# OSU-Bee-Lab/buzzdetect

Measured on AMD Instinct MI355X. Metric: yamnet_windows_per_s, higher is better.
Workload: dtype f32 (split-f16x3 MFMA products, f32 accumulate)

## Files before the change

buzzdetect_amd/csrc/sepchip.hip:

```cpp
#include "bd_device.h"

namespace bd {

namespace {

constexpr int kChipHalfBytes = 97 * 64;
constexpr int kChipSlotBytes = 2 * kChipHalfBytes;

constexpr int kChipMaxLayers = 5;
struct ChipChain {
    const float* dw_w[kChipMaxLayers];
    const float* dw_b[kChipMaxLayers];
    const _Float16* whi[kChipMaxLayers];
    const _Float16* wlo[kChipMaxLayers];
    const float* pw_u[kChipMaxLayers];
    const float* pw_b[kChipMaxLayers];
    const float* ndw_w;
    const _Float16 *w7hi, *w7lo;
    const float *u7, *b7;
};
template <typename T>
__device__ __forceinline__ const T* chain_ptr(int field, int li) {
    typedef const __attribute__((address_space(4))) unsigned long long* kptr;
    const kptr ka = (kptr)__builtin_amdgcn_kernarg_segment_ptr();
    return reinterpret_cast<const T*>(ka[field * kChipMaxLayers + li]);
}
static_assert(sizeof(ChipChain) == (6 * kChipMaxLayers + 5) * 8, "six tables of five pointers + five");

template <bool PLAIN, int NSLOT, bool TRACE = false, bool NDW = false, bool PLANES = false, bool PW7 = false>
__global__ __launch_bounds__(512, 2) void sep_chip_kernel(const ChipChain ch, const float* X, float* Y, int nl,
                                                           long long M, unsigned* __restrict__ range_flag,
                                                           unsigned long long* __restrict__ dbg = nullptr, int tune = 0) {
    static_assert(NSLOT >= 9 && NSLOT <= 16, "ring size");
    constexpr int K = 512, KQ = K / 16;
    constexpr int NPEND = 16 - NSLOT;
    extern __shared__ __attribute__((aligned(16))) char sm[];
    const int tid = threadIdx.x;
    const int lane = tid & 63;
    const int wc = __builtin_amdgcn_readfirstlane(tid >> 6);
    const int frow = lane & 31, fh = lane >> 5;
    const long long m0 = (long long)blockIdx.x * 96;
    float rmax = 0.0f;
    int tsn = 0;
#define CHIP_TS()                                                                                         \
    if constexpr (TRACE) {                                                                                \
        if (blockIdx.x == 0 && lane == 0 && (wc == 0 || wc == 5) && tsn < 64)                             \
            dbg[(wc == 5 ? 64 : 0) + tsn] = __builtin_amdgcn_s_memtime();                                 \
        ++tsn;                                                                                            \
    }
    CHIP_TS()

    const int wb0 = fh * (48 * 64 + 64) + ((frow >> 3) << 4) + 2 * (frow & 7);
    const int ra0 = frow * 64 + ((fh ^ ((frow >> 2) & 3)) << 4);
    const int ra1 = ra0 + 2048 + (frow >= 16 ? 64 : 0);
    const unsigned lane16 = lane * 16, c4 = frow * 4;

    f32x16 acc[3][2];
    unsigned pend[48], out0[48];

#define CHIP_DW(J, ST, TAPS)                                                                              \
    {                                                                                                     \
        float wt[9];                                                                                      \
        _Pragma("unroll") for (int t = 0; t < 9; ++t)                                                     \
            wt[t] = __builtin_bit_cast(float, __builtin_amdgcn_raw_buffer_load_b32(TAPS, c4, (t * K + 32 * (ST)) * 4, 0)); \
        const float shift = __builtin_bit_cast(float, __builtin_amdgcn_raw_buffer_load_b32(TAPS, c4, (9 * K + 32 * (ST)) * 4, 0)); \
        _Pragma("unroll") for (int y = 0; y < 6; ++y)                                                     \
            _Pragma("unroll") for (int x = 0; x < 4; ++x) {                                               \
                v2f a = {shift, shift};                                                                   \
                _Pragma("unroll") for (int kh = 0; kh < 3; ++kh)                                          \
                    _Pragma("unroll") for (int kw = 0; kw < 3; ++kw) {                                    \
                        const int iy = y + kh - 1, ix = x + kw - 1;                                       \
                        if (iy < 0 || iy >= 6 || ix < 0 || ix >= 4) continue;                             \
                        a = __builtin_elementwise_fma(in2[iy][ix], v2f{wt[kh * 3 + kw], wt[kh * 3 + kw]}, a); \
                    }                                                                                     \
                _Pragma("unroll") for (int w = 0; w < 2; ++w) {                                           \
                    const float v = fmaxf(w ? a.y : a.x, 0.0f);                                           \
                    unsigned pk = (unsigned)__builtin_bit_cast(unsigned short, (_Float16)v);              \
                     \
                     \
                    asm volatile("v_fma_mixhi_f16 %0, %0, -1.0, %2 op_sel:[0,0,0] op_sel_hi:[1,0,0]\n\tv_max_f32 %1, %1, %2" \
                                 : "+v"(pk), "+v"(rmax) : "v"(v));                                        \
                    const int rl = 24 * w + 4 * y + x;                                \
                    if ((J) == 1) pend[rl] = pk;                                                          \
                    else out0[rl] = pk;                                                                   \
                }                                                                                         \
            }                                                                                             \
    }
#define CHIP_PUBLISH()                                                                                    \
    {                                                                                                     \
        int wbl = wb0;        \
        asm volatile("" : "+v"(wbl));                       \
        char* const slot0 = sm + wc * kChipSlotBytes;                                                     \
        _Pragma("unroll") for (int rl = 0; rl < 48; ++rl) CHIP_PUT(slot0, rl, out0[rl])                   \
        if (wc + 8 < NSLOT) {                                                \
            char* const slot1 = sm + (wc + 8) * kChipSlotBytes;                                           \
            _Pragma("unroll") for (int rl = 0; rl < 48; ++rl) CHIP_PUT(slot1, rl, pend[rl])               \
        }                                                                                                 \
    }
#define CHIP_PUT(SLOT, RL, PK)                                                                            \
    {                                                                                                     \
        char* const p_ = (SLOT) + (wbl ^ ((((RL) >> 2) & 3) << 4)) + (RL) * 64;                           \
        *reinterpret_cast<unsigned short*>(p_) = (unsigned short)(PK);                                    \
        *reinterpret_cast<unsigned short*>(p_ + kChipHalfBytes) = (unsigned short)((PK) >> 16);           \
    }
#define CHIP_TAPS_RSRC(DW_W) __builtin_amdgcn_make_buffer_rsrc(const_cast<float*>(DW_W), 0, 10 * K * 4, 0x00020000)

    auto k_loop = [&](auto kq_c, const _Float16* const Wfhi, const _Float16* const Wflo) __attribute__((always_inline)) {
        constexpr int KQL = decltype(kq_c)::value;
        constexpr int NS = KQL / 2;
        constexpr int NP = NS > NSLOT ? NS - NSLOT : 0;
        static_assert(NP == 0 || NP == NPEND, "a layer of K = 512 or one that fits the ring");
        const __amdgpu_buffer_rsrc_t bhr = __builtin_amdgcn_make_buffer_rsrc(const_cast<_Float16*>(Wfhi), 0, 16 * KQL * K * 2, 0x00020000);
        const __amdgpu_buffer_rsrc_t blr = __builtin_amdgcn_make_buffer_rsrc(const_cast<_Float16*>(Wflo), 0, 16 * KQL * K * 2, 0x00020000);
        const int btile = wc * (KQL * 1024);
        constexpr int jstep = 8 * KQL * 1024;
        f16x8 bh0[2], bl0[2], bh1[2], bl1[2];
#define CHIP_LB(R, B, Q, J) B[J] = __builtin_bit_cast(f16x8, __builtin_amdgcn_raw_buffer_load_b128(R, lane16, btile + (J) * jstep + (Q) * 1024, 0));
#define CHIP_BLOAD(BH, BL, Q) { CHIP_LB(bhr, BH, Q, 0) CHIP_LB(blr, BL, Q, 0) CHIP_LB(bhr, BH, Q, 1) CHIP_LB(blr, BL, Q, 1) }
        CHIP_BLOAD(bh0, bl0, 0)
        __syncthreads();
        CHIP_TS()

        float zero;
        asm volatile("v_mov_b32 %0, 0" : "=v"(zero));
#pragma unroll
        for (int i = 0; i < 3; ++i)
#pragma unroll
            for (int j = 0; j < 2; ++j)
#pragma unroll
                for (int r = 0; r < 16; ++r) acc[i][j][r] = zero;
#define CHIP_LAH(A, S, I) A = *reinterpret_cast<const f16x8*>(abase + (((I) == 1 ? ra1 : ra0) ^ ((S) << 5)) + ((I) == 2 ? 4096 + 64 : 0));
#define CHIP_LAL(A, S, I) A = *reinterpret_cast<const f16x8*>(abase + (((I) == 1 ? ra1 : ra0) ^ ((S) << 5)) + ((I) == 2 ? 4096 + 64 : 0) + kChipHalfBytes);
#define CHIP_MF(I, J, A, B) acc[I][J] = __builtin_amdgcn_mfma_f32_32x32x16_f16(A, B, acc[I][J], 0, 0, 0);
#define CHIP_SB __builtin_amdgcn_sched_barrier(0);
#define CHIP_NOP
#define CHIP_STEP(I, AH, AL, BH, BL, M1, M2, M3, M4, M5, M6)                                              \
    if constexpr (!PLAIN) {                                                                               \
        CHIP_MF(I, 0, AL, BH[0]) M1 CHIP_SB                                                               \
        CHIP_MF(I, 0, AH, BL[0]) M2 CHIP_SB                                                               \
    } else {                                                                                              \
        M1 M2                                                                                             \
    }                                                                                                     \
    CHIP_MF(I, 0, AH, BH[0]) M3 CHIP_SB                                                                   \
    if constexpr (!PLAIN) {                                                                               \
        CHIP_MF(I, 1, AL, BH[1]) M4 CHIP_SB                                                               \
        CHIP_MF(I, 1, AH, BL[1]) M5 CHIP_SB                                                               \
    } else {                                                                                              \
        M4 M5                                                                                             \
    }                                                                                                     \
    CHIP_MF(I, 1, AH, BH[1]) M6 CHIP_SB
#define CHIP_STAGES(FROM, TO)                                                                             \
    if ((FROM) < (TO)) {                                                                                  \
        f16x8 ah0, al0, ah1, al1, ah2, al2;                                                               \
        const char* abase = sm + ((FROM) < NSLOT ? (FROM) : (FROM) - NSLOT) * kChipSlotBytes;             \
        CHIP_LAH(ah0, 0, 0) CHIP_LAL(al0, 0, 0) CHIP_LAH(ah1, 0, 1) CHIP_LAL(al1, 0, 1)                   \
        _Pragma("nounroll") for (int kk = (FROM); kk < (TO); ++kk) {                                      \
            const int q1 = 2 * kk + 1, q2 = 2 * kk + 2 < KQL ? 2 * kk + 2 : 0;     \
            const char* const anext = sm + (kk + 1 < (TO) ? (kk + 1 < NSLOT ? kk + 1 : kk + 1 - NSLOT) : (kk < NSLOT ? kk : kk - NSLOT)) * kChipSlotBytes; \
            CHIP_STEP(0, ah0, al0, bh0, bl0, CHIP_LB(bhr, bh1, q1, 0), CHIP_LB(blr, bl1, q1, 0), CHIP_LB(bhr, bh1, q1, 1),  \
                      CHIP_LB(blr, bl1, q1, 1), CHIP_LAH(ah2, 0, 2), CHIP_LAL(al2, 0, 2))                 \
            CHIP_STEP(1, ah1, al1, bh0, bl0, CHIP_LAH(ah0, 1, 0), CHIP_LAL(al0, 1, 0), CHIP_NOP, CHIP_NOP, CHIP_NOP, CHIP_NOP) \
            CHIP_STEP(2, ah2, al2, bh0, bl0, CHIP_LAH(ah1, 1, 1), CHIP_LAL(al1, 1, 1), CHIP_LB(blr, bl0, q2, 0),            \
                      CHIP_LB(bhr, bh0, q2, 0), CHIP_NOP, CHIP_LB(blr, bl0, q2, 1))                       \
            CHIP_STEP(0, ah0, al0, bh1, bl1, CHIP_LB(bhr, bh0, q2, 1), CHIP_LAH(ah2, 1, 2), CHIP_LAL(al2, 1, 2), CHIP_NOP, CHIP_NOP, CHIP_NOP) \
            abase = anext;          \
            CHIP_STEP(1, ah1, al1, bh1, bl1, CHIP_LAH(ah0, 0, 0), CHIP_LAL(al0, 0, 0), CHIP_NOP, CHIP_NOP, CHIP_NOP, CHIP_NOP) \
            CHIP_STEP(2, ah2, al2, bh1, bl1, CHIP_LAH(ah1, 0, 1), CHIP_LAL(al1, 0, 1), CHIP_NOP, CHIP_NOP, CHIP_NOP, CHIP_NOP) \
        }                                                                                                 \
    }
        CHIP_STAGES(0, NP)
        CHIP_TS()
        if constexpr (NP > 0) {
            __syncthreads();
            CHIP_TS()
            if (wc >= 8 - NPEND) {
                char* const slot = sm + (wc + 8 - NSLOT) * kChipSlotBytes;
                int wbl = wb0;
                asm volatile("" : "+v"(wbl));
#pragma unroll
                for (int rl = 0; rl < 48; ++rl) CHIP_PUT(slot, rl, pend[rl])
            }
        }
        CHIP_TS()
        if constexpr (NP > 0) __syncthreads();
        CHIP_TS()
        CHIP_STAGES(NP, NS)
        CHIP_TS()
#undef CHIP_STAGES
#undef CHIP_STEP
#undef CHIP_BLOAD
#undef CHIP_LB
#undef CHIP_LAH
#undef CHIP_LAL
#undef CHIP_MF
#undef CHIP_SB
#undef CHIP_NOP
    };

    auto next_layer = [&](const float* const taps_w, const float* const pu, const float* const pb) __attribute__((always_inline)) {
        const __amdgpu_buffer_rsrc_t taps = CHIP_TAPS_RSRC(taps_w);
        const __amdgpu_buffer_rsrc_t pur = __builtin_amdgcn_make_buffer_rsrc(const_cast<float*>(pu), 0, K * 4, 0x00020000);
        const __amdgpu_buffer_rsrc_t pbr = __builtin_amdgcn_make_buffer_rsrc(const_cast<float*>(pb), 0, K * 4, 0x00020000);
#pragma unroll
        for (int j = 0; j < 2; ++j) {
            const int st = j ? wc + 8 : wc;
            const float u = __builtin_bit_cast(float, __builtin_amdgcn_raw_buffer_load_b32(pur, c4, 128 * st, 0));
            const float b = __builtin_bit_cast(float, __builtin_amdgcn_raw_buffer_load_b32(pbr, c4, 128 * st, 0));
            float ev[12][4];
#pragma unroll
            for (int q = 0; q < 6; ++q)
#pragma unroll
                for (int x = 0; x < 4; ++x) {
                    const float a01 = fmaxf(fmaf(acc[q >> 2][j][4 * (q & 3) + x], u, b), 0.0f);
                    const float a23 = fmaxf(fmaf(acc[(q + 6) >> 2][j][4 * ((q + 6) & 3) + x], u, b), 0.0f);
                    const auto r = __builtin_amdgcn_permlane32_swap(__builtin_bit_cast(unsigned, a01),
                                                                    __builtin_bit_cast(unsigned, a23), false, false);
                    ev[2 * q][x] = __builtin_bit_cast(float, (unsigned)r[0]);
                    ev[2 * q + 1][x] = __builtin_bit_cast(float, (unsigned)r[1]);
                }
            v2f in2[6][4];
#pragma unroll
            for (int y = 0; y < 6; ++y)
#pragma unroll
                for (int x = 0; x < 4; ++x) in2[y][x] = v2f{ev[y][x], ev[6 + y][x]};
            if (j == 0) CHIP_DW(0, st, taps)
            else CHIP_DW(1, st, taps)
            CHIP_TS()
        }
        __syncthreads();
        CHIP_TS()
        CHIP_PUBLISH()
    };

    const long long rows_left = M - m0;
    const unsigned tile_bytes = (unsigned)(rows_left < 96 ? rows_left : 96) * (K * 4);
    if constexpr (PW7) {
        const long long w0 = m0 / 24, wleft = M / 24 - w0;
        const __amdgpu_buffer_rsrc_t pr = __builtin_amdgcn_make_buffer_rsrc(
            const_cast<char*>(reinterpret_cast<const char*>(X)) + (size_t)w0 * kDw7PlaneBytes, 0,
            (unsigned)(wleft < 4 ? wleft : 4) * kDw7PlaneBytes, 0x00020000);
        constexpr int kPieces = 8 * kChipSlotBytes / 1024;
        static_assert(kPieces * 1024 == 8 * kChipSlotBytes && 8 * kChipSlotBytes <= NSLOT * kChipSlotBytes, "whole pieces");
#pragma unroll
        for (int t = 0; t < (kPieces + 7) / 8; ++t) {
            const int n = 8 * t + wc;
            if (n >= kPieces) break;
            const int c = 64 * n + lane;
            const int s = c / (kChipSlotBytes / 16), cs = c - s * (kChipSlotBytes / 16);
            const int h = cs >= kChipHalfBytes / 16 ? 1 : 0;
            const int o = (cs - h * (kChipHalfBytes / 16)) * 16;
            const bool skew = o >= 48 * 64 && o < 49 * 64;
            const int rho = o < 48 * 64 ? o >> 6 : (o - 64) >> 6;
            const int p = (o >> 4) & 3, w = rho / 24;
            const unsigned src = (unsigned)(w * kDw7PlaneBytes + s * (kDw7PlaneBytes / 8) + h * (kDw7PlaneBytes / 16) +
                                            (rho - 24 * w) * 64 + ((p ^ ((rho >> 2) & 3)) << 4));
            const unsigned off = skew || (PLAIN && h) ? 0x7ffffff0u : src;
            __builtin_amdgcn_raw_ptr_buffer_load_lds(pr, (__attribute__((address_space(3))) void*)(sm + n * 1024), 16, off, 0, 0, 0);
        }
        asm volatile("s_waitcnt vmcnt(0)" ::: "memory");
        CHIP_TS()
        k_loop(std::integral_constant<int, 16>{}, ch.w7hi, ch.w7lo);
        next_layer(ch.dw_w[0], ch.u7, ch.b7);
    } else {
        const __amdgpu_buffer_rsrc_t xrs = __builtin_amdgcn_make_buffer_rsrc(const_cast<float*>(X) + (size_t)m0 * K, 0, tile_bytes, 0x00020000);
        const __amdgpu_buffer_rsrc_t taps0 = CHIP_TAPS_RSRC(ch.dw_w[0]);
        const unsigned xo = (48u * fh * K) * 4 + c4;
#pragma unroll
        for (int j = 0; j < 2; ++j) {
            const int st = j ? wc + 8 : wc;
            v2f in2[6][4];
#pragma unroll
            for (int y = 0; y < 6; ++y)
#pragma unroll
                for (int x = 0; x < 4; ++x) {
                    in2[y][x].x = __builtin_bit_cast(float, __builtin_amdgcn_raw_buffer_load_b32(xrs, xo, ((4 * y + x) * K + 32 * st) * 4, 0));
                    in2[y][x].y = __builtin_bit_cast(float, __builtin_amdgcn_raw_buffer_load_b32(xrs, xo, ((24 + 4 * y + x) * K + 32 * st) * 4, 0));
                }
            if (j == 0) CHIP_DW(0, st, taps0)
            else CHIP_DW(1, st, taps0)
            CHIP_TS()
            __builtin_amdgcn_sched_barrier(0);
        }
        CHIP_PUBLISH()
    }

    for (int li = 0; li < nl; ++li) {
        k_loop(std::integral_constant<int, KQ>{}, chain_ptr<_Float16>(2, li), chain_ptr<_Float16>(3, li));
        if (li + 1 == nl) break;
        next_layer(chain_ptr<float>(0, li + 1), chain_ptr<float>(4, li), chain_ptr<float>(5, li));
    }
#undef CHIP_DW
#undef CHIP_PUBLISH
#undef CHIP_TAPS_RSRC
#undef CHIP_PUT

    {
        const __amdgpu_buffer_rsrc_t pur = __builtin_amdgcn_make_buffer_rsrc(const_cast<float*>(chain_ptr<float>(4, nl - 1)), 0, K * 4, 0x00020000);
        const __amdgpu_buffer_rsrc_t pbr = __builtin_amdgcn_make_buffer_rsrc(const_cast<float*>(chain_ptr<float>(5, nl - 1)), 0, K * 4, 0x00020000);
        if constexpr (!NDW) {
            const __amdgpu_buffer_rsrc_t yrs = __builtin_amdgcn_make_buffer_rsrc(Y + (size_t)m0 * K, 0, tile_bytes, 0x00020000);
            const unsigned yo = (4u * fh * K) * 4 + c4;
#pragma unroll
            for (int j = 0; j < 2; ++j) {
                const int st = j ? wc + 8 : wc;
                const float u = __builtin_bit_cast(float, __builtin_amdgcn_raw_buffer_load_b32(pur, c4, 128 * st, 0));
                const float b = __builtin_bit_cast(float, __builtin_amdgcn_raw_buffer_load_b32(pbr, c4, 128 * st, 0));
#pragma unroll
                for (int i = 0; i < 3; ++i)
#pragma unroll
                    for (int r = 0; r < 16; ++r)
                        __builtin_amdgcn_raw_buffer_store_b32(__builtin_bit_cast(unsigned, fmaxf(fmaf(acc[i][j][r], u, b), 0.0f)), yrs, yo,
                                                              ((32 * i + 8 * (r >> 2) + (r & 3)) * K + 32 * st) * 4, 0);
            }
        } else {
            const __amdgpu_buffer_rsrc_t yrs = __builtin_amdgcn_make_buffer_rsrc(Y + (size_t)(m0 / 4) * K, 0, tile_bytes / 4, 0x00020000);
            _Float16* const yh = reinterpret_cast<_Float16*>(Y);
            const __amdgpu_buffer_rsrc_t yhr = __builtin_amdgcn_make_buffer_rsrc(yh + (size_t)(m0 / 4) * K, 0, tile_bytes / 8, 0x00020000);
            const __amdgpu_buffer_rsrc_t ylr = __builtin_amdgcn_make_buffer_rsrc(yh + (size_t)(M / 4 + m0 / 4) * K, 0, tile_bytes / 8, 0x00020000);
            const __amdgpu_buffer_rsrc_t ntaps = __builtin_amdgcn_make_buffer_rsrc(const_cast<float*>(ch.ndw_w), 0, 10 * K * 4, 0x00020000);
            const unsigned yo = (12u * fh * K) * 4 + c4;
#pragma unroll
            for (int j = 0; j < 2; ++j) {
                const int st = j ? wc + 8 : wc;
                const float u = __builtin_bit_cast(float, __builtin_amdgcn_raw_buffer_load_b32(pur, c4, 128 * st, 0));
                const float b = __builtin_bit_cast(float, __builtin_amdgcn_raw_buffer_load_b32(pbr, c4, 128 * st, 0));
                float wt[9];
#pragma unroll
                for (int t = 0; t < 9; ++t)
                    wt[t] = __builtin_bit_cast(float, __builtin_amdgcn_raw_buffer_load_b32(ntaps, c4, (t * K + 32 * st) * 4, 0));
                const float shift = __builtin_bit_cast(float, __builtin_amdgcn_raw_buffer_load_b32(ntaps, c4, (9 * K + 32 * st) * 4, 0));
                float ev[12][4];
#pragma unroll
                for (int q = 0; q < 6; ++q)
#pragma unroll
                    for (int x = 0; x < 4; ++x) {
                        const float a01 = fmaxf(fmaf(acc[q >> 2][j][4 * (q & 3) + x], u, b), 0.0f);
                        const float a23 = fmaxf(fmaf(acc[(q + 6) >> 2][j][4 * ((q + 6) & 3) + x], u, b), 0.0f);
                        const auto r = __builtin_amdgcn_permlane32_swap(__builtin_bit_cast(unsigned, a01),
                                                                        __builtin_bit_cast(unsigned, a23), false, false);
                        ev[2 * q][x] = __builtin_bit_cast(float, (unsigned)r[0]);
                        ev[2 * q + 1][x] = __builtin_bit_cast(float, (unsigned)r[1]);
                    }
#pragma unroll
                for (int oy = 0; oy < 3; ++oy)
#pragma unroll
                    for (int ox = 0; ox < 2; ++ox) {
                        v2f a = {shift, shift};
#pragma unroll
                        for (int kh = 0; kh < 3; ++kh)
#pragma unroll
                            for (int kw = 0; kw < 3; ++kw) {
                                const int iy = 2 * oy + kh, ix = 2 * ox + kw;
                                if (iy >= 6 || ix >= 4) continue;
                                a = __builtin_elementwise_fma(v2f{ev[iy][ix], ev[6 + iy][ix]}, v2f{wt[kh * 3 + kw], wt[kh * 3 + kw]}, a);
                            }
#pragma unroll
                        for (int w = 0; w < 2; ++w) {
                            const float o = fmaxf(w ? a.y : a.x, 0.0f);
                            if constexpr (PLANES) {
                                unsigned pk = (unsigned)__builtin_bit_cast(unsigned short, (_Float16)o);
                                asm volatile("v_fma_mixhi_f16 %0, %0, -1.0, %2 op_sel:[0,0,0] op_sel_hi:[1,0,0]\n\tv_max_f32 %1, %1, |%2|"
                                             : "+v"(pk), "+v"(rmax) : "v"(o));
                                __builtin_amdgcn_raw_buffer_store_b16((unsigned short)pk, yhr, yo >> 1, ((6 * w + 2 * oy + ox) * K + 32 * st) * 2, 0);
                                if constexpr (!PLAIN)
                                    __builtin_amdgcn_raw_buffer_store_b16((unsigned short)(pk >> 16), ylr, yo >> 1,
                                                                          ((6 * w + 2 * oy + ox) * K + 32 * st) * 2, 0);
                            } else {
                                __builtin_amdgcn_raw_buffer_store_b32(__builtin_bit_cast(unsigned, o), yrs, yo,
                                                                      ((6 * w + 2 * oy + ox) * K + 32 * st) * 4, 0);
                            }
                        }
                    }
            }
        }
    }
    range_report(rmax, range_flag);
    if constexpr (TRACE) asm volatile("s_waitcnt vmcnt(0)" ::: "memory");
    CHIP_TS()
#undef CHIP_TS
}

template <bool PLAIN, bool NDW, bool PLANES = false, bool PW7 = false>
void launch_chip(const float* in, float* out, const SepLayer* L, int nl, long long M, const float* ndw_w, hipStream_t stream,
                 const SepLayer* L7 = nullptr) {
    ChipChain ch{};
    if (L7) {
        ch.w7hi = static_cast<const _Float16*>(L7->pw_fhi);
        ch.w7lo = static_cast<const _Float16*>(L7->pw_flo);
        ch.u7 = L7->pw_u;
        ch.b7 = L7->pw_b;
    }
    for (int i = 0; i < nl; ++i) {
        ch.dw_w[i] = dw_w_of(L[i]);
        ch.dw_b[i] = dw_b_of(L[i]);
        ch.whi[i] = static_cast<const _Float16*>(L[i].pw_fhi);
        ch.wlo[i] = static_cast<const _Float16*>(L[i].pw_flo);
        ch.pw_u[i] = L[i].pw_u;
        ch.pw_b[i] = L[i].pw_b;
    }
    ch.ndw_w = ndw_w;
    constexpr int NSLOT = 13;
    constexpr int lds = NSLOT * kChipSlotBytes;
    static_assert(lds <= 160 * 1024, "the ring must fit the CU's LDS");
    allow_dynamic_lds<&sep_chip_kernel<PLAIN, NSLOT, false, NDW, PLANES, PW7>>(lds);
    const long long tiles = (M + 95) / 96;
    int tune = 0;
#ifdef BD_KERNEL_TRACE
    if (const char* tn = getenv("BD_CHIP_TUNE")) tune = atoi(tn);
    if (traced_launch(
            '7', &sep_chip_kernel<PLAIN, NSLOT, true, NDW, PLANES, PW7>, lds, stream, 64, 5, nullptr,
            [&](unsigned long long* dbg) {
                hipLaunchKernelGGL((sep_chip_kernel<PLAIN, NSLOT, true, NDW, PLANES, PW7>), dim3((unsigned)tiles), dim3(512), lds, stream, ch, in, out, nl,
                                   M, L[0].range_flag, dbg, tune);
            },
            "on-chip run, wave %d, %d layers%s: cycles between stamps (start | %s | per layer: B1, stages 0-2, B2, pend, B3, stages 3-15, "
            "[dw j0, dw j1, B4] | stores):",
            nl, PW7 ? " + pointwise 7" : "", PW7 ? "DMA, B1, -, -, -, stages 0-7, dw j0, dw j1, B4" : "dw0 j0 j1"))
        return;
#endif
    hipLaunchKernelGGL((sep_chip_kernel<PLAIN, NSLOT, false, NDW, PLANES, PW7>), dim3((unsigned)tiles), dim3(512), lds, stream, ch, in, out, nl, M,
                       L[0].range_flag, (unsigned long long*)nullptr, tune);
}

}

static bool launch_separable_chip(const float* in, float* out, int windows, const SepLayer* L, int nl, hipStream_t stream,
                                  const SepLayer* next, bool planes) {
    if (planes && !next) return false;
    if (nl < 1 || nl > kChipMaxLayers) return false;
    for (int i = 0; i < nl; ++i)
        if (dw_b_of(L[i]) != dw_w_of(L[i]) + 9 * 512) return false;
    if (next && (dw_b_of(*next) != dw_w_of(*next) + 9 * 512 || next->cin != 512 || next->stride != 2 || in == out)) return false;
    const long long M = (long long)windows * 24;
    const float* nw = next ? dw_w_of(*next) : nullptr;
    if (planes) {
        if (L[0].pw_mode == 2) launch_chip<true, true, true>(in, out, L, nl, M, nw, stream);
        else launch_chip<false, true, true>(in, out, L, nl, M, nw, stream);
        return true;
    }
    if (L[0].pw_mode == 2) {
        if (next) launch_chip<true, true>(in, out, L, nl, M, nw, stream);
        else launch_chip<true, false>(in, out, L, nl, M, nw, stream);
    } else {
        if (next) launch_chip<false, true>(in, out, L, nl, M, nw, stream);
        else launch_chip<false, false>(in, out, L, nl, M, nw, stream);
    }
    return true;
}

int launch_separable_run_next_dw(const float* a, float* b, int windows, const SepLayer* L, int max_layers, hipStream_t stream,
                                 bool planes) {
    int n = 0;
    while (n < 5 && n + 1 < max_layers) {
        const SepLayer& l = L[n];
        if (l.stride != 1 || l.cin != 512 || l.cout != 512 || l.h_out != 6 || l.w_out != 4 || l.pw_mode != L[0].pw_mode) return 0;
        ++n;
        if (L[n].stride != 1) break;
    }
    if (n < 2 || n > 5 || n >= max_layers || L[n].stride != 2 || L[n].cin != 512 || windows <= 0 || (long long)windows * 24 >= (1LL << 31))
        return 0;
    return launch_separable_chip(a, b, windows, L, n, stream, &L[n], planes) ? n : 0;
}

bool separable_chip_pw7_supported(const SepLayer& L7, const SepLayer* L, int nl, const SepLayer& next, int windows) {
    if (windows <= 0 || (long long)windows * 24 >= (1LL << 31) || nl < 1 || nl > kChipMaxLayers) return false;
    if (L7.cin != 256 || L7.cout != 512 || L7.h_out != 6 || L7.w_out != 4 || L7.pw_mode == 0 || !L7.pw_fhi || !L7.pw_flo)
        return false;
    for (int i = 0; i < nl; ++i)
        if (L[i].stride != 1 || L[i].cin != 512 || L[i].cout != 512 || L[i].h_out != 6 || L[i].w_out != 4 ||
            L[i].pw_mode != L7.pw_mode || dw_b_of(L[i]) != dw_w_of(L[i]) + 9 * 512)
            return false;
    return next.stride == 2 && next.cin == 512 && dw_b_of(next) == dw_w_of(next) + 9 * 512;
}

bool launch_separable_chip_pw7(const void* in, float* out, int windows, const SepLayer& L7, const SepLayer* L, int nl,
                               const SepLayer& next, hipStream_t stream) {
    if (!separable_chip_pw7_supported(L7, L, nl, next, windows) || in == out) return false;
    const float* const X = static_cast<const float*>(in);
    const long long M = (long long)windows * 24;
    if (L7.pw_mode == 2) launch_chip<true, true, true, true>(X, out, L, nl, M, dw_w_of(next), stream, &L7);
    else launch_chip<false, true, true, true>(X, out, L, nl, M, dw_w_of(next), stream, &L7);
    return true;
}

}
```

buzzdetect_amd/csrc/sepmid.hip:

```cpp
#include "bd_device.h"

#include <type_traits>

namespace bd {

namespace {

constexpr int kHalfA = 97 * 64;
constexpr int kSlotA = 2 * kHalfA;
constexpr int kHalf7 = 48 * 64;
constexpr int kSlot7 = 2 * kHalf7;
constexpr int kOffA7 = 8 * kSlotA;
constexpr int kMidLds = kOffA7 + 8 * kSlot7 + 1024;
static_assert(kMidLds <= 160 * 1024, "one workgroup per CU");
constexpr int kStage7 = kDw7PlaneBytes / 8;
constexpr int kMidLdsDw7 = kOffA7 + 8 * kStage7;
static_assert(kStage7 == 2 * 24 * 64, "[hi, lo][24 rows][32 channels] f16");

struct MidArgs {
    const _Float16 *w5h, *w5l, *w6h, *w6l, *w7h, *w7l;
    const float *u5, *b5, *u6, *b6, *u7, *b7;
    const float *dw6, *dw7;
};

#define MID_RSRC(P, BYTES) __builtin_amdgcn_make_buffer_rsrc(const_cast<void*>(static_cast<const void*>(P)), 0, (BYTES), 0x00020000)
#define MID_LD32(R, VOFF, SOFF) __builtin_bit_cast(float, __builtin_amdgcn_raw_buffer_load_b32(R, VOFF, SOFF, 0))
#define MID_LD128(R, VOFF, SOFF) __builtin_bit_cast(f16x8, __builtin_amdgcn_raw_buffer_load_b128(R, VOFF, SOFF, 0))

template <bool PLAIN, bool TRACE, bool DW7OUT = false>
__global__ __launch_bounds__(512, 2) void sep_mid_kernel(const MidArgs a, const float* __restrict__ X, float* __restrict__ Y, int windows,
                                                          unsigned* __restrict__ range_flag, unsigned long long* __restrict__ dbg) {
    extern __shared__ __attribute__((aligned(16))) char sm[];
    const int tid = threadIdx.x, lane = tid & 63;
    const int wc = __builtin_amdgcn_readfirstlane(tid >> 6);
    const int frow = lane & 31, fh = lane >> 5;
    float rmax = 0.0f;
    int tsn = 0;
#define MID_TS()                                                                                          \
    if constexpr (TRACE) {                                                                                \
        if (blockIdx.x == 0 && lane == 0 && (wc == 0 || wc == 5) && tsn < 64)                             \
            dbg[(wc == 5 ? 64 : 0) + tsn] = __builtin_amdgcn_s_memtime();                                 \
        ++tsn;                                                                                            \
    }
    const int wb0 = fh * (48 * 64 + 64) + ((frow >> 3) << 4) + 2 * (frow & 7);
    const int wb7 = fh * 128 + ((frow >> 3) << 4) + 2 * (frow & 7);
    const int ra0 = frow * 64 + ((fh ^ ((frow >> 2) & 3)) << 4);
    const int ra1 = ra0 + 2048 + (frow >= 16 ? 64 : 0);
    const unsigned lane16 = lane * 16, c4 = frow * 4;

#define MID_PUT(BASE, RL, PK)                                                                             \
    {                                                                                                     \
        char* const p_ = (BASE) + (wbl ^ ((((RL) >> 2) & 3) << 4)) + (RL) * 64;                           \
        *reinterpret_cast<unsigned short*>(p_) = (unsigned short)(PK);                                    \
        *reinterpret_cast<unsigned short*>(p_ + kHalfA) = (unsigned short)((PK) >> 16);                   \
    }
#define MID_SPLIT(V, PK)                                                                                  \
    unsigned PK = (unsigned)__builtin_bit_cast(unsigned short, (_Float16)(V));                            \
    asm volatile("v_fma_mixhi_f16 %0, %0, -1.0, %2 op_sel:[0,0,0] op_sel_hi:[1,0,0]\n\tv_max_f32 %1, %1, |%2|"   \
                 : "+v"(PK), "+v"(rmax) : "v"(V));
#define MID_MMA(ACC, AH, AL, BHV, BLV)                                                                    \
    if constexpr (!PLAIN) {                                                                               \
        ACC = __builtin_amdgcn_mfma_f32_32x32x16_f16(AL, BHV, ACC, 0, 0, 0);                              \
        ACC = __builtin_amdgcn_mfma_f32_32x32x16_f16(AH, BLV, ACC, 0, 0, 0);                              \
    }                                                                                                     \
    ACC = __builtin_amdgcn_mfma_f32_32x32x16_f16(AH, BHV, ACC, 0, 0, 0);

#define MID_TILE_TO_MAP(ACC, U, B, EV)                                                                    \
    _Pragma("unroll") for (int q = 0; q < 6; ++q)                                                         \
        _Pragma("unroll") for (int e = 0; e < 4; ++e) {                                                   \
            const float lo_ = fmaxf(fmaf(ACC[q >> 2][4 * (q & 3) + e], U, B), 0.0f);                      \
            const float hi_ = fmaxf(fmaf(ACC[(q + 6) >> 2][4 * ((q + 6) & 3) + e], U, B), 0.0f);          \
            const auto r_ = __builtin_amdgcn_permlane32_swap(__builtin_bit_cast(unsigned, lo_), __builtin_bit_cast(unsigned, hi_), false, false); \
            EV[2 * q][e] = __builtin_bit_cast(float, (unsigned)r_[0]);                                    \
            EV[2 * q + 1][e] = __builtin_bit_cast(float, (unsigned)r_[1]);                                \
        }
#define MID_HALO(EV, LH, RH)                                                                              \
    _Pragma("unroll") for (int y = 0; y < 12; ++y) {                                                      \
        const auto r_ = __builtin_amdgcn_permlane32_swap(__builtin_bit_cast(unsigned, EV[y][0]), __builtin_bit_cast(unsigned, EV[y][3]), false, false); \
        LH[y] = fh ? __builtin_bit_cast(float, (unsigned)r_[0]) : 0.0f;        \
        RH[y] = fh ? 0.0f : __builtin_bit_cast(float, (unsigned)r_[1]);        \
    }

#define MID_ROW_PAIRS(EV, LH, RH, IN2)                                                                    \
    _Pragma("unroll") for (int c = 0; c < 6; ++c) {                                                       \
        _Pragma("unroll") for (int r = 0; r < 6; ++r)                                                     \
            IN2[1 + r][c] = c == 0 ? v2f{LH[r], LH[r + 6]} : c == 5 ? v2f{RH[r], RH[r + 6]} : v2f{EV[r][c - 1], EV[r + 6][c - 1]}; \
        IN2[0][c] = v2f{0.0f, c == 0 ? LH[5] : c == 5 ? RH[5] : EV[5][c - 1]};                            \
        IN2[7][c] = v2f{c == 0 ? LH[6] : c == 5 ? RH[6] : EV[6][c - 1], 0.0f};                            \
    }

    float vin[24];
    auto fetch_window = [&](int win) {
        const __amdgpu_buffer_rsrc_t xr = MID_RSRC(X + (size_t)win * 96 * 128, 96 * 128 * 4);
        const int st = wc & 3, rl0 = 24 * (wc >> 2);
        const unsigned vo = (4u * fh * 128) * 4 + c4;
#pragma unroll
        for (int t = 0; t < 24; ++t) {
            const int rl = rl0 + t;
            vin[t] = MID_LD32(xr, vo, ((8 * (rl >> 2) + (rl & 3)) * 128 + 32 * st) * 4);
        }
    };
    f16x8 b7h[3][2], b7l[3][2];
    const __amdgpu_buffer_rsrc_t r7h = MID_RSRC(a.w7h, 256 * 512 * 2), r7l = MID_RSRC(a.w7l, 256 * 512 * 2);
    auto window_to_a7 = [&](auto half_c, auto last_c, int win, int win_next) {
        constexpr int HALF = decltype(half_c)::value;
        constexpr bool LAST = decltype(last_c)::value;
        {
            const int st = wc & 3;
            int wbl = wb0;
            asm volatile("" : "+v"(wbl));
            char* const slot = sm + st * kSlotA;
            if (wc < 4) {
#pragma unroll
                for (int t = 0; t < 24; ++t) {
                    MID_SPLIT(vin[t], pk)
                    MID_PUT(slot, t, pk)
                }
            } else {
#pragma unroll
                for (int t = 0; t < 24; ++t) {
                    MID_SPLIT(vin[t], pk)
                    MID_PUT(slot, 24 + t, pk)
                }
            }
        }
        f16x8 bh[3], bl[3];
        const __amdgpu_buffer_rsrc_t r5h = MID_RSRC(a.w5h, 128 * 256 * 2), r5l = MID_RSRC(a.w5l, 128 * 256 * 2);
#pragma unroll
        for (int q = 0; q < 2; ++q) {
            bh[q] = MID_LD128(r5h, lane16, (wc * 8 + q) * 1024);
            bl[q] = MID_LD128(r5l, lane16, (wc * 8 + q) * 1024);
        }
        __syncthreads();
        MID_TS()
        f32x16 acc[3];
        float zero;
        asm volatile("v_mov_b32 %0, 0" : "=v"(zero));
#pragma unroll
        for (int i = 0; i < 3; ++i)
#pragma unroll
            for (int r = 0; r < 16; ++r) acc[i][r] = zero;
        {
            constexpr int KQ = 8;
#pragma unroll
            for (int q = 0; q < KQ; ++q) {
                if (q + 2 < KQ) {
                    bh[(q + 2) % 3] = MID_LD128(r5h, lane16, (wc * KQ + q + 2) * 1024);
                    bl[(q + 2) % 3] = MID_LD128(r5l, lane16, (wc * KQ + q + 2) * 1024);
                }
                const char* const ab = sm + (q >> 1) * kSlotA;
#pragma unroll
                for (int i = 0; i < 3; ++i) {
                    const char* const ap = ab + ((i == 1 ? ra1 : ra0) ^ ((q & 1) << 5)) + (i == 2 ? 4096 + 64 : 0);
                    const f16x8 ah = *reinterpret_cast<const f16x8*>(ap), al = *reinterpret_cast<const f16x8*>(ap + kHalfA);
                    MID_MMA(acc[i], ah, al, bh[q % 3], bl[q % 3])
                }
            }
        }
        MID_TS()
        const __amdgpu_buffer_rsrc_t r6h = MID_RSRC(a.w6h, 256 * 256 * 2), r6l = MID_RSRC(a.w6l, 256 * 256 * 2);
        {
            unsigned out6[48];
            {
                const __amdgpu_buffer_rsrc_t ur = MID_RSRC(a.u5, 1024), br = MID_RSRC(a.b5, 1024), tr = MID_RSRC(a.dw6, 10 * 256 * 4);
                const float u = MID_LD32(ur, c4, 128 * wc), b = MID_LD32(br, c4, 128 * wc);
                float wt[9];
#pragma unroll
                for (int t = 0; t < 9; ++t) wt[t] = MID_LD32(tr, c4, (t * 256 + 32 * wc) * 4);
                const float shift = MID_LD32(tr, c4, (9 * 256 + 32 * wc) * 4);
                float ev[12][4], lh[12], rh[12];
                MID_TILE_TO_MAP(acc, u, b, ev)
                MID_HALO(ev, lh, rh)
                v2f in2[8][6];
                MID_ROW_PAIRS(ev, lh, rh, in2)
#pragma unroll
                for (int y = 0; y < 6; ++y)
#pragma unroll
                    for (int e = 0; e < 4; ++e) {
                        v2f sacc = {shift, shift};
#pragma unroll
                        for (int kh = 0; kh < 3; ++kh)
#pragma unroll
                            for (int kw = 0; kw < 3; ++kw)
                                sacc = __builtin_elementwise_fma(in2[y + kh][e + kw], v2f{wt[kh * 3 + kw], wt[kh * 3 + kw]}, sacc);
#pragma unroll
                        for (int w = 0; w < 2; ++w) {
                            const float o = fmaxf(w ? sacc.y : sacc.x, 0.0f);
                            MID_SPLIT(o, pk)
                            out6[4 * (y + 6 * w) + e] = pk;
                        }
                    }
            }
            __syncthreads();
            MID_TS()
#pragma unroll
            for (int q = 0; q < 2; ++q) {
                bh[q] = MID_LD128(r6h, lane16, (wc * 16 + q) * 1024);
                bl[q] = MID_LD128(r6l, lane16, (wc * 16 + q) * 1024);
            }
            int wbl = wb0;
            asm volatile("" : "+v"(wbl));
            char* const slot = sm + wc * kSlotA;
#pragma unroll
            for (int rl = 0; rl < 48; ++rl) MID_PUT(slot, rl, out6[rl])
        }
        __syncthreads();
        MID_TS()
        asm volatile("v_mov_b32 %0, 0" : "=v"(zero));
#pragma unroll
        for (int i = 0; i < 3; ++i)
#pragma unroll
            for (int r = 0; r < 16; ++r) acc[i][r] = zero;
        {
            constexpr int KQ = 16;
#pragma unroll
            for (int q = 0; q < KQ; ++q) {
                if (q + 2 < KQ) {
                    bh[(q + 2) % 3] = MID_LD128(r6h, lane16, (wc * KQ + q + 2) * 1024);
                    bl[(q + 2) % 3] = MID_LD128(r6l, lane16, (wc * KQ + q + 2) * 1024);
                }
                const char* const ab = sm + (q >> 1) * kSlotA;
#pragma unroll
                for (int i = 0; i < 3; ++i) {
                    const char* const ap = ab + ((i == 1 ? ra1 : ra0) ^ ((q & 1) << 5)) + (i == 2 ? 4096 + 64 : 0);
                    const f16x8 ah = *reinterpret_cast<const f16x8*>(ap), al = *reinterpret_cast<const f16x8*>(ap + kHalfA);
                    MID_MMA(acc[i], ah, al, bh[q % 3], bl[q % 3])
                }
            }
        }
        MID_TS()
        if (win_next >= 0) fetch_window(win_next);
        {
            const __amdgpu_buffer_rsrc_t ur = MID_RSRC(a.u6, 1024), br = MID_RSRC(a.b6, 1024), tr = MID_RSRC(a.dw7, 10 * 256 * 4);
            const float u = MID_LD32(ur, c4, 128 * wc), b = MID_LD32(br, c4, 128 * wc);
            float wt[9];
#pragma unroll
            for (int t = 0; t < 9; ++t) wt[t] = MID_LD32(tr, c4, (t * 256 + 32 * wc) * 4);
            const float shift = MID_LD32(tr, c4, (9 * 256 + 32 * wc) * 4);
            float ev[12][4], lh[12], rh[12];
            MID_TILE_TO_MAP(acc, u, b, ev)
            MID_HALO(ev, lh, rh)
            int wbl = wb7;
            asm volatile("" : "+v"(wbl));
            char* const slot = sm + kOffA7 + wc * kSlot7;
            char* const stg = sm + kOffA7 + wc * kStage7;
            v2f in2[8][6];
            MID_ROW_PAIRS(ev, lh, rh, in2)
#pragma unroll
            for (int oy = 0; oy < 3; ++oy)
#pragma unroll
                for (int j = 0; j < 2; ++j) {
                    v2f sacc = {shift, shift};
#pragma unroll
                    for (int kh = 0; kh < 3; ++kh)
#pragma unroll
                        for (int kw = 0; kw < 3; ++kw)
                            sacc = __builtin_elementwise_fma(in2[1 + 2 * oy + kh][1 + 2 * j + kw], v2f{wt[kh * 3 + kw], wt[kh * 3 + kw]}, sacc);
#pragma unroll
                    for (int w = 0; w < 2; ++w) {
                        const int oyw = oy + 3 * w;
                        const float o = fmaxf(w ? sacc.y : sacc.x, 0.0f);
                        MID_SPLIT(o, pk)
                        if constexpr (DW7OUT) {
                            char* const p_ = stg + (4 * oyw + 2 * fh + j) * 64 + 2 * frow;
                            *reinterpret_cast<unsigned short*>(p_) = (unsigned short)pk;
                            if constexpr (!PLAIN) *reinterpret_cast<unsigned short*>(p_ + kStage7 / 2) = (unsigned short)(pk >> 16);
                        } else {
                            char* const p_ = slot + (wbl ^ (((6 * HALF + oyw) & 3) << 4)) + (24 * HALF + 4 * oyw + j) * 64;
                            *reinterpret_cast<unsigned short*>(p_) = (unsigned short)pk;
                            *reinterpret_cast<unsigned short*>(p_ + kHalf7) = (unsigned short)(pk >> 16);
                        }
                    }
                }
            if constexpr (DW7OUT) {
                typedef __attribute__((address_space(1))) char* gchar;
                asm volatile("" ::: "memory");
                const gchar dst = (gchar)Y + (size_t)win * kDw7PlaneBytes + wc * kStage7 + lane * 16;
#pragma unroll
                for (int t = 0; t < 3; ++t) {
                    if (PLAIN && (t == 2 || (t == 1 && lane >= 32))) continue;
                    const v4f v = *reinterpret_cast<const v4f*>(stg + t * 1024 + lane * 16);
                    asm volatile("global_store_dwordx4 %0, %1, off\n\ts_nop 2" : : "v"(dst + t * 1024), "v"(v) : "memory");
                }
            }
        }
        if constexpr (LAST) {
#pragma unroll
            for (int q = 0; q < 2; ++q)
#pragma unroll
                for (int j = 0; j < 2; ++j) {
                    b7h[q][j] = MID_LD128(r7h, lane16, ((wc + 8 * j) * 16 + q) * 1024);
                    b7l[q][j] = MID_LD128(r7l, lane16, ((wc + 8 * j) * 16 + q) * 1024);
                }
        }
        __syncthreads();
        MID_TS()
    };
    auto layer7 = [&](auto nw_c, int win) {
        constexpr int NW = decltype(nw_c)::value;
        f32x16 c7[NW][2];
        float zero;
        asm volatile("v_mov_b32 %0, 0" : "=v"(zero));
#pragma unroll
        for (int i = 0; i < NW; ++i)
#pragma unroll
            for (int j = 0; j < 2; ++j)
#pragma unroll
                for (int r = 0; r < 16; ++r) c7[i][j][r] = zero;
        constexpr int KQ = 16;
        const int ra7 = frow * 64 + ((fh ^ ((frow >> 2) & 3)) << 4);
#pragma unroll
        for (int q = 0; q < KQ; ++q) {
            if (q + 2 < KQ) {
#pragma unroll
                for (int j = 0; j < 2; ++j) {
                    b7h[(q + 2) % 3][j] = MID_LD128(r7h, lane16, ((wc + 8 * j) * KQ + q + 2) * 1024);
                    b7l[(q + 2) % 3][j] = MID_LD128(r7l, lane16, ((wc + 8 * j) * KQ + q + 2) * 1024);
                }
            }
#pragma unroll
            for (int i = 0; i < NW; ++i) {
                const char* const ap = sm + kOffA7 + (q >> 1) * kSlot7 + (ra7 ^ ((q & 1) << 5)) + i * 2048;
                const f16x8 ah = *reinterpret_cast<const f16x8*>(ap), al = *reinterpret_cast<const f16x8*>(ap + kHalf7);
#pragma unroll
                for (int j = 0; j < 2; ++j) { MID_MMA(c7[i][j], ah, al, b7h[q % 3][j], b7l[q % 3][j]) }
            }
        }
        MID_TS()
        const __amdgpu_buffer_rsrc_t ur = MID_RSRC(a.u7, 2048), br = MID_RSRC(a.b7, 2048);
        const __amdgpu_buffer_rsrc_t yr = MID_RSRC(Y + (size_t)win * 24 * 512, NW * 24 * 512 * 4);
        const unsigned yo = (4u * fh * 512) * 4 + c4;
#pragma unroll
        for (int j = 0; j < 2; ++j) {
            const float u = MID_LD32(ur, c4, 128 * (wc + 8 * j)), b = MID_LD32(br, c4, 128 * (wc + 8 * j));
#pragma unroll
            for (int i = 0; i < NW; ++i)
#pragma unroll
                for (int r = 0; r < (NW == 1 ? 12 : 16); ++r)
                    __builtin_amdgcn_raw_buffer_store_b32(__builtin_bit_cast(unsigned, fmaxf(fmaf(c7[i][j][r], u, b), 0.0f)), yr, yo,
                                                          ((32 * i + 8 * (r >> 2) + (r & 3)) * 512 + 32 * (wc + 8 * j)) * 4, 0);
        }
        MID_TS()
    };

    MID_TS()
    const int w_begin = (int)(((long long)blockIdx.x * windows) / gridDim.x);
    const int w_end = (int)(((long long)(blockIdx.x + 1) * windows) / gridDim.x);
    if (w_begin < w_end) fetch_window(w_begin);
    if constexpr (DW7OUT) {
        for (int win = w_begin; win < w_end; ++win)
            window_to_a7(std::integral_constant<int, 0>{}, std::false_type{}, win, win + 1 < w_end ? win + 1 : -1);
    } else for (int win = w_begin; win < w_end; win += 2) {
        const bool two = win + 1 < w_end;
        if (two) {
            window_to_a7(std::integral_constant<int, 0>{}, std::false_type{}, win, win + 1);
            window_to_a7(std::integral_constant<int, 1>{}, std::true_type{}, win + 1, win + 2 < w_end ? win + 2 : -1);
            layer7(std::integral_constant<int, 2>{}, win);
        } else {
            window_to_a7(std::integral_constant<int, 0>{}, std::true_type{}, win, -1);
            layer7(std::integral_constant<int, 1>{}, win);
        }
    }
    range_report(rmax, range_flag);
#undef MID_TS
#undef MID_PUT
#undef MID_SPLIT
#undef MID_MMA
#undef MID_TILE_TO_MAP
#undef MID_HALO
}

template <bool PLAIN, bool DW7OUT>
void launch_mid(const float* in, float* out, int windows, const SepLayer& L5, const SepLayer& L6, const SepLayer& L7, hipStream_t stream) {
    constexpr int lds = DW7OUT ? kMidLdsDw7 : kMidLds;
    MidArgs a{};
    a.w5h = static_cast<const _Float16*>(L5.pw_fhi);
    a.w5l = static_cast<const _Float16*>(L5.pw_flo);
    a.w6h = static_cast<const _Float16*>(L6.pw_fhi);
    a.w6l = static_cast<const _Float16*>(L6.pw_flo);
    a.w7h = static_cast<const _Float16*>(L7.pw_fhi);
    a.w7l = static_cast<const _Float16*>(L7.pw_flo);
    a.u5 = L5.pw_u; a.b5 = L5.pw_b;
    a.u6 = L6.pw_u; a.b6 = L6.pw_b;
    a.u7 = L7.pw_u; a.b7 = L7.pw_b;
    a.dw6 = dw_w_of(L6);
    a.dw7 = dw_w_of(L7);
    allow_dynamic_lds<&sep_mid_kernel<PLAIN, false, DW7OUT>>(lds);
    int grid = cu_count();
    if (grid > windows) grid = windows;
#ifdef BD_KERNEL_TRACE
    if (traced_launch(
            '8', &sep_mid_kernel<PLAIN, true, DW7OUT>, lds, stream, 64, 5, nullptr,
            [&](unsigned long long* dbg) {
                hipLaunchKernelGGL((sep_mid_kernel<PLAIN, true, DW7OUT>), dim3(grid), dim3(512), lds, stream, a, in, out, windows, L5.range_flag, dbg);
            },
            "mid run, wave %d: cycles between stamps (per window: A5+B1, K5, dw6+Bx, publish+B2, K6, %s):",
            DW7OUT ? "dw7 + its planes stored" : "dw7+B3; per pair: K7, stores"))
        return;
#endif
    hipLaunchKernelGGL((sep_mid_kernel<PLAIN, false, DW7OUT>), dim3(grid), dim3(512), lds, stream, a, in, out, windows, L5.range_flag,
                       (unsigned long long*)nullptr);
}

}

namespace {
bool mid_shapes_ok(const SepLayer& L5, const SepLayer& L6, const SepLayer& L7) {
    if (L5.cin != 128 || L5.cout != 256 || L5.h_out != 12 || L5.w_out != 8 || L6.cin != 256 || L6.cout != 256 || L6.stride != 1 ||
        L6.h_out != 12 || L6.w_out != 8 || L7.cin != 256 || L7.cout != 512 || L7.stride != 2 || L7.h_out != 6 || L7.w_out != 4)
        return false;
    if (L5.pw_mode == 0 || L6.pw_mode != L5.pw_mode || L7.pw_mode != L5.pw_mode) return false;
    return dw_b_of(L6) == dw_w_of(L6) + 9 * 256 && dw_b_of(L7) == dw_w_of(L7) + 9 * 256;
}
}

bool launch_separable_mid(const float* in, float* out, int windows, const SepLayer& L5, const SepLayer& L6, const SepLayer& L7,
                          hipStream_t stream) {
    if (windows <= 0 || in == out || !mid_shapes_ok(L5, L6, L7)) return false;
    if (L5.pw_mode == 2) launch_mid<true, false>(in, out, windows, L5, L6, L7, stream);
    else launch_mid<false, false>(in, out, windows, L5, L6, L7, stream);
    return true;
}

bool separable_mid_planes_supported(const SepLayer& L5, const SepLayer& L6, const SepLayer& L7) { return mid_shapes_ok(L5, L6, L7); }

bool launch_separable_mid_planes(const float* in, void* out, int windows, const SepLayer& L5, const SepLayer& L6, const SepLayer& L7,
                                 hipStream_t stream) {
    if (windows <= 0 || in == out || !mid_shapes_ok(L5, L6, L7)) return false;
    float* const Y = static_cast<float*>(out);
    if (L5.pw_mode == 2) launch_mid<true, true>(in, Y, windows, L5, L6, L7, stream);
    else launch_mid<false, true>(in, Y, windows, L5, L6, L7, stream);
    return true;
}

}
```

Baseline: 2.084 million.

## Vectorize mid-kernel window fetch to 128-bit loads and split barrier by wave group

The mid kernel now loads each input window with six 128-bit buffer loads per lane instead of 24 scalar loads, splits four values at once into f16 hi/lo, and writes them to LDS as 8-byte stores through a new swizzled address (wb5). This is meant to cut memory instructions and LDS store count in the window-to-A staging. The chip kernel also moves the barrier for waves 4-7 to before their depthwise work, so the two wave groups stagger around one barrier. That staggering only works if both groups still reach the same number of barriers, and the new LDS layout has to match what the readers expect.

```diff
diff --git a/buzzdetect_amd/csrc/sepchip.hip b/buzzdetect_amd/csrc/sepchip.hip
--- a/buzzdetect_amd/csrc/sepchip.hip
+++ b/buzzdetect_amd/csrc/sepchip.hip
@@ -201,6 +201,7 @@
         const __amdgpu_buffer_rsrc_t taps = CHIP_TAPS_RSRC(taps_w);
         const __amdgpu_buffer_rsrc_t pur = __builtin_amdgcn_make_buffer_rsrc(const_cast<float*>(pu), 0, K * 4, 0x00020000);
         const __amdgpu_buffer_rsrc_t pbr = __builtin_amdgcn_make_buffer_rsrc(const_cast<float*>(pb), 0, K * 4, 0x00020000);
+        if (wc >= 4) __syncthreads();
 #pragma unroll
         for (int j = 0; j < 2; ++j) {
             const int st = j ? wc + 8 : wc;
@@ -227,7 +228,7 @@
             else CHIP_DW(1, st, taps)
             CHIP_TS()
         }
-        __syncthreads();
+        if (wc < 4) __syncthreads();
         CHIP_TS()
         CHIP_PUBLISH()
     };
diff --git a/buzzdetect_amd/csrc/sepmid.hip b/buzzdetect_amd/csrc/sepmid.hip
--- a/buzzdetect_amd/csrc/sepmid.hip
+++ b/buzzdetect_amd/csrc/sepmid.hip
@@ -43,6 +43,8 @@
         ++tsn;                                                                                            \
     }
     const int wb0 = fh * (48 * 64 + 64) + ((frow >> 3) << 4) + 2 * (frow & 7);
+    const int wb5 = (frow >> 3) * kSlotA + fh * 64 + (((frow & 7) >> 1) << 4) + 8 * (frow & 1);
+    static_assert((kSlotA & 0x70) == 0 && kHalfA % 8 == 0, "the slot bits of wb5 are its own; 8-byte writes");
     const int wb7 = fh * 128 + ((frow >> 3) << 4) + 2 * (frow & 7);
     const int ra0 = frow * 64 + ((fh ^ ((frow >> 2) & 3)) << 4);
     const int ra1 = ra0 + 2048 + (frow >= 16 ? 64 : 0);
@@ -89,16 +91,11 @@
         IN2[7][c] = v2f{c == 0 ? LH[6] : c == 5 ? RH[6] : EV[6][c - 1], 0.0f};                            \
     }
 
-    float vin[24];
+    v4f vin[6];
     auto fetch_window = [&](int win) {
         const __amdgpu_buffer_rsrc_t xr = MID_RSRC(X + (size_t)win * 96 * 128, 96 * 128 * 4);
-        const int st = wc & 3, rl0 = 24 * (wc >> 2);
-        const unsigned vo = (4u * fh * 128) * 4 + c4;
-#pragma unroll
-        for (int t = 0; t < 24; ++t) {
-            const int rl = rl0 + t;
-            vin[t] = MID_LD32(xr, vo, ((8 * (rl >> 2) + (rl & 3)) * 128 + 32 * st) * 4);
-        }
+#pragma unroll
+        for (int t = 0; t < 6; ++t) vin[t] = __builtin_bit_cast(v4f, __builtin_amdgcn_raw_buffer_load_b128(xr, lane16, (6 * wc + t) * 1024, 0));
     };
     f16x8 b7h[3][2], b7l[3][2];
     const __amdgpu_buffer_rsrc_t r7h = MID_RSRC(a.w7h, 256 * 512 * 2), r7l = MID_RSRC(a.w7l, 256 * 512 * 2);
@@ -106,22 +103,18 @@
         constexpr int HALF = decltype(half_c)::value;
         constexpr bool LAST = decltype(last_c)::value;
         {
-            const int st = wc & 3;
-            int wbl = wb0;
+            int wbl = wb5;
             asm volatile("" : "+v"(wbl));
-            char* const slot = sm + st * kSlotA;
-            if (wc < 4) {
-#pragma unroll
-                for (int t = 0; t < 24; ++t) {
-                    MID_SPLIT(vin[t], pk)
-                    MID_PUT(slot, t, pk)
-                }
-            } else {
-#pragma unroll
-                for (int t = 0; t < 24; ++t) {
-                    MID_SPLIT(vin[t], pk)
-                    MID_PUT(slot, 24 + t, pk)
-                }
+#pragma unroll
+            for (int t = 0; t < 6; ++t) {
+                const int pe = 12 * wc + 2 * t;
+                const int y = pe >> 3, xh = (pe >> 2) & 1;
+                rmax = range_of(rmax, vin[t]);
+                f16x4 hi, lo;
+                split_f16(vin[t], hi, lo);
+                char* const p_ = sm + (wbl ^ ((y & 3) << 4)) + (48 * xh + 4 * y + (pe & 2)) * 64 + xh * 64;
+                *reinterpret_cast<f16x4*>(p_) = hi;
+                *reinterpret_cast<f16x4*>(p_ + kHalfA) = lo;
             }
         }
         f16x8 bh[3], bl[3];
```

After: 2.107 million (median of 6 runs). 1.01x the previous value.
